# JuanLuisGonzalez/FAL_net

Measured on AMD Instinct MI355X. Metric: stereo-pairs/sec Stage-1 step @256x512 N=49, higher is better.
Workload: dtype bf16; 1 GPU; Stage-1 training step (BASELINE configs[1]), batch 8/GPU, 256x512, N=49, seeded weights, seeded VGG19; global_batch=8, parallelism=dp1, launch=eager launches, recorded sequences issued by falnet_replay (C)

## Files before the change

### fal_net_amd/_build.py

```python
import os
import subprocess
import sys
from concurrent.futures import ThreadPoolExecutor

HERE = os.path.dirname(os.path.abspath(__file__))
CSRC = os.path.join(HERE, "csrc")
OBJ = os.path.join(HERE, "csrc", "_obj")
LIB = os.path.join(HERE, "libfalnet_hip.so")
SOURCES = ["api.cpp", "replay.cpp", "med_head.hip", "med_head2.hip", "med_sweep.hip", "med_stats.hip", "compact.hip", "losses.hip", "elementwise.hip", "data.hip", "augment_batch.hip", "dump.hip", "metrics.hip", "velo.hip", "lidar.hip", "sort.hip", "sparsify.hip", "wgrad_rows.hip", "wgrad_wave.hip", "wgrad.hip", "pack.hip", "conv_wave.hip", "conv_dma.hip", "conv.hip"]
HIPCC = os.environ.get("HIPCC", "/opt/rocm/bin/hipcc")
FLAGS = ["--offload-arch=gfx950", "-O3", "-fPIC", "-std=c++17", "-Wall", "-Wno-unused-function"]
FILE_FLAGS = {"med_head.hip": ["-fno-slp-vectorize"], "med_head2.hip": ["-fno-slp-vectorize"], "med_sweep.hip": ["-fno-slp-vectorize"],
              "med_stats.hip": ["-fno-slp-vectorize"],
              "dump.hip": ["-ffp-contract=off"],
              "metrics.hip": ["-ffp-contract=off"], "augment_batch.hip": ["-ffp-contract=off"], "velo.hip": ["-ffp-contract=off"],
              "lidar.hip": ["-ffp-contract=off"], "sparsify.hip": ["-ffp-contract=off"]}


def _stale(out, deps):
    if not os.path.exists(out):
        return True
    t = os.path.getmtime(out)
    return any(os.path.getmtime(d) > t for d in deps)


def build_ab(tag="ab", defines=(), verbose=True, raw=()):
    obj_dir = os.path.join(CSRC, "_obj_" + tag)
    os.makedirs(obj_dir, exist_ok=True)
    flags = FLAGS + ["-DFALNET_AB"] + ["-D" + d for d in defines]
    lib = os.path.join(HERE, f"libfalnet_hip_{tag}.so")

    def run(src):
        cmd = [HIPCC] + flags + FILE_FLAGS.get(src, []) + list(raw) + (["-x", "hip"] if src.endswith(".hip") else []) + ["-c", os.path.join(CSRC, src), "-o", os.path.join(obj_dir, src + ".o")]
        if verbose:
            print(" ".join(cmd), flush=True)
        subprocess.run(cmd, check=True)
    with ThreadPoolExecutor(max_workers=4) as ex:
        list(ex.map(run, SOURCES))
    subprocess.run([HIPCC, "--offload-arch=gfx950", "-shared", "-fPIC", "-o", lib] + [os.path.join(obj_dir, s + ".o") for s in SOURCES], check=True)
    return lib


def build(force=False, verbose=True):
    os.makedirs(OBJ, exist_ok=True)
    headers = [os.path.join(CSRC, "common.h"), os.path.join(CSRC, "conv_epilogue.h"), os.path.join(HERE, "..", "include", "falnet_hip.h")]
    jobs = []
    for src in SOURCES:
        path = os.path.join(CSRC, src)
        obj = os.path.join(OBJ, src + ".o")
        if force or _stale(obj, [path] + headers):
            cmd = [HIPCC] + FLAGS + FILE_FLAGS.get(src, []) + (["-x", "hip"] if src.endswith(".hip") else []) + ["-c", path, "-o", obj]
            jobs.append(cmd)

    def run(cmd):
        if verbose:
            print(" ".join(cmd), flush=True)
        subprocess.run(cmd, check=True)

    with ThreadPoolExecutor(max_workers=4) as ex:
        list(ex.map(run, jobs))
    objs = [os.path.join(OBJ, s + ".o") for s in SOURCES]
    if force or jobs or _stale(LIB, objs):
        run([HIPCC, "--offload-arch=gfx950", "-shared", "-fPIC", "-o", LIB] + objs)
    return LIB


if __name__ == "__main__":
    if "--ab" in sys.argv:
        rest = [a for a in sys.argv[sys.argv.index("--ab") + 1:]]
        tag = next((a for a in rest if not a.startswith("-")), "ab")
        print(build_ab(tag, [a[2:] for a in rest if a.startswith("-D")], raw=[a for a in rest if a.startswith("-") and not a.startswith("-D")]))
    else:
        build(force="--force" in sys.argv)
        print(LIB)
```

### fal_net_amd/csrc/conv.hip

```cpp
#include <limits.h>
#include <stdlib.h>
#include <type_traits>
#include "common.h"
#include "conv_epilogue.h"

#define CONV_THREADS 256
#define CONV_BM 128
#define ROWB 64
#define ROWP 80

template <typename T> struct KC;
template <> struct KC<float> { static constexpr int value = 16; };
template <> struct KC<bf16_t> { static constexpr int value = 32; };
template <> struct KC<f16_t> { static constexpr int value = 32; };

template <typename T, int MT, int NT, typename RowOff, typename PoolOff = NoPool>
__device__ __forceinline__ void epilogue_nhwc(const falnet_conv_t& p, f32x16 (&acc)[MT][NT], float* stage, int nbase, int lane,
                                              RowOff rowoff, PoolOff pooloff = PoolOff()) {
    constexpr bool POOL = !std::is_same<PoolOff, NoPool>::value;
    constexpr int PITCHF = NT * 32 + 4;
    constexpr int CS = NT * 4;
    constexpr int RPP = 64 / CS;
    constexpr int PASSES = 32 / RPP;
    const int r = lane & 31, h = lane >> 5;
// ... 1382 lines not shown
    }
    C3_STAMP(5);
    asm volatile("s_waitcnt vmcnt(0)" ::: "memory");
    C3_STAMP(6);
}
#undef C3_STAMP

template <typename T, bool SWAP>
static void launch_conv(const falnet_conv_t& p, int bn, dim3 grid, hipStream_t st) {
    if (bn == 128)
        hipLaunchKernelGGL(HIP_KERNEL_NAME(conv_igemm_kernel<T, 128, SWAP>), grid, dim3(CONV_THREADS), 0, st, p);
    else if (bn == 64)
        hipLaunchKernelGGL(HIP_KERNEL_NAME(conv_igemm_kernel<T, 64, SWAP>), grid, dim3(CONV_THREADS), 0, st, p);
    else
        hipLaunchKernelGGL(HIP_KERNEL_NAME(conv_igemm_kernel<T, 32, SWAP>), grid, dim3(CONV_THREADS), 0, st, p);
}

static bool falnet_mfma16_enabled() {
    static const bool on = [] { const char* e = falnet_ab_env("FALNET_MFMA16"); return !(e && e[0] == '0'); }();
    return on;
}

enum class ConvFamily {
    Gather,
    Patch,
    WeightStationary,
    Dma,
    S2fDma,
    Up2Dma,
    Deep,
    Dma2,
    Dma16,
    Up2d,
    Wave32,
    Wave64p,
};
struct ConvChoice {
    ConvFamily family;
    int bn, kcb, tps, adb, th, nwaves, flip, swap;
};

static bool g_disable_patch = [] { const char* e = falnet_ab_env("FALNET_DISABLE_PATCH"); return e && e[0] == '1'; }();
static int g_patch_kcb = [] { const char* e = falnet_ab_env("FALNET_PATCH_KCB"); return e ? atoi(e) : 128; }();


bool falnet_conv_dma_applicable(const falnet_conv_t& p, int min_oh);
int falnet_conv_dma_launch(const falnet_conv_t& p, int flip, hipStream_t st, int th);
bool falnet_conv_dma2_applicable(const falnet_conv_t& p, int th);
int falnet_conv_dma2_launch(const falnet_conv_t& p, int flip, hipStream_t st, int th);
int falnet_conv_dma16_launch(const falnet_conv_t& p, int flip, hipStream_t st, int th);
bool falnet_conv_up2_dma_applicable(const falnet_conv_t& p);
int falnet_conv_up2_dma_launch(const falnet_conv_t& p, hipStream_t st);
bool falnet_conv_wave32_applicable(const falnet_conv_t& p);
int falnet_conv_wave32_launch(const falnet_conv_t& p, int flip, hipStream_t st);
bool falnet_conv_wave64p_applicable(const falnet_conv_t& p);
int falnet_conv_wave64p_launch(const falnet_conv_t& p, int flip, hipStream_t st);
bool falnet_conv_up2d_applicable(const falnet_conv_t& p);
int falnet_conv_up2d_launch(const falnet_conv_t& p, hipStream_t st);
bool falnet_conv_deep_applicable(const falnet_conv_t& p);
int falnet_conv_deep_launch(const falnet_conv_t& p, hipStream_t st);
int falnet_conv_deep_mtiles(const falnet_conv_t& p);
bool falnet_conv_s2d_dma_applicable(const falnet_conv_t* d, int n);
int falnet_conv_s2d_dma_launch(const falnet_conv_t* d, hipStream_t st);
bool falnet_conv_s2f_dma_applicable(const falnet_conv_t& p);
int falnet_conv_s2f_dma_launch(const falnet_conv_t& p, hipStream_t st);

static int choose_conv_kernel(const falnet_conv_t& p, ConvChoice& c) {
    const bool planar = p.out_layout == FALNET_OUT_PLANAR_F32;
    int ctot = 0;
    for (int s = 0; s < p.nsrc; ++s) ctot += p.src[s].C;
    bool dense3x3 = p.ntaps == 9 && p.isy == 1 && p.isx == 1 && p.osy == 1 && p.osx == 1 && p.ooy == 0 && p.oox == 0 &&
                    p.TH == p.OH && p.TW == p.OW && p.TH == p.IH && p.TW == p.IW && p.TW >= 16;
    int flip = -1;
    if (dense3x3 && p.w_taps == 9) {
        bool fwd = true, bwd = true;
        for (int t = 0; t < 9; ++t) {
            const int sp = (p.tap_dy[t] + 1) * 3 + (p.tap_dx[t] + 1);
            if (p.tap_dy[t] < -1 || p.tap_dy[t] > 1 || p.tap_dx[t] < -1 || p.tap_dx[t] > 1) fwd = bwd = false;
            fwd = fwd && p.tap_w[t] == sp;
            bwd = bwd && p.tap_w[t] == 8 - sp;
        }
        flip = fwd ? 0 : (bwd ? 1 : -1);
    }
    dense3x3 = dense3x3 && flip >= 0;
    const int esz = p.dtype == FALNET_F32 ? 4 : 2;
    bool c128 = true;
    for (int s = 0; s < p.nsrc; ++s) c128 = c128 && (p.src[s].C % (128 / esz) == 0);
    int variant = p.variant;
    int forced_bn = 0;
    if (variant == 11 || variant == 12) {
        forced_bn = variant == 11 ? 32 : 64;
        if (p.w_rows % forced_bn != 0 || p.pool_out) {
            falnet_set_error("conv2d: variant %d (gather, %d channels per workgroup) not applicable to this launch", variant, forced_bn);
            return -2;
        }
        variant = 1;
    }
    if (p.pool_code && !(variant == 23 && p.dtype != FALNET_F32 && p.pool_out && p.pool_mode == 0 && !planar && p.OH % 2 == 0 && p.OW % 2 == 0 &&
                         p.Cout % 32 == 0 && p.out_cstride % 32 == 0)) {
        falnet_set_error("conv2d: pool_code (argmax codes of the fused max pool) needs variant 23, a 16-bit type, pool_out with pool_mode 0, an NHWC "
                         "launch with even OH / OW and whole 32-channel groups (variant %d, dtype %d, pool_mode %d)", p.variant, p.dtype, p.pool_mode);
        return -2;
    }
    if (g_disable_patch) variant = 1;
    switch (variant) {
        case 0: case 1: case 2: case 3: case 4: case 5: case 6: case 7: case 8: case 9: case 10:
        case 13: case 15: case 16: case 17: case 18: case 19: case 20: case 21: case 22: case 23: case 24: case 25: case 26: case 27: case 29:
            break;
        default:
            falnet_set_error("conv2d: unknown variant %d", variant);
            return -1;
    }
    if (variant == 19) {
        if (!falnet_conv_deep_applicable(p)) {
            falnet_set_error("conv2d: variant 19 needs a 16-bit nine-tap stride-1/2 launch on maps of at most 128 positions (128 %% (TH TW) == 0), dense NHWC output, "
                             "w_rows %% 64 == 0, ksplit = cin_total / 32 or / 64 (a multiple of 4), scratch for the partial tiles and the split-K workspace");
            return -2;
        }
        c.flip = 0;
        c.swap = 0;
        c.family = ConvFamily::Deep;
        c.bn = 64; c.kcb = p.ksplit * 32 == p.cin_total ? 1 : 2; c.tps = 9; c.adb = 1; c.th = 0; c.nwaves = falnet_conv_deep_mtiles(p);
        return 0;
    }
    if (variant == 15) {
        if (!falnet_conv_s2f_dma_applicable(p)) {
            falnet_set_error("conv2d: variant 15 needs a canonical 16-bit 3x3 stride-2 pad-1 NHWC launch (>= 8 x 32 outputs) with sources at the input size");
            return -2;
        }
        c.flip = 0;
        c.swap = 0;
        c.family = ConvFamily::S2fDma;
        c.bn = 64; c.kcb = 32; c.tps = 9; c.adb = 1; c.th = 8; c.nwaves = 8;
        return 0;
    }
    if (variant == 29) {
        if (!(dense3x3 && falnet_conv_wave64p_applicable(p))) {
            falnet_set_error("conv2d: variant 29 needs a 16-bit dense 3x3 stride-1 launch over ONE 64-channel source at the launch size, planar f32 output of <= 4 channels, no addend / activation-gradient operand / pool / split-K");
            return -2;
        }
        c.flip = flip;
        c.swap = 0;
        c.family = ConvFamily::Wave64p;
        c.bn = 16; c.kcb = 32; c.tps = 9; c.adb = 1; c.th = 1; c.nwaves = 8;
        return 0;
    }
    if (variant == 27) {
        if (!(dense3x3 && falnet_conv_wave32_applicable(p))) {
            falnet_set_error("conv2d: variant 27 needs a 16-bit dense 3x3 stride-1 NHWC launch over ONE 32-channel source at the launch size with a 32-row packed weight, no pool / split-K");
            return -2;
        }
        c.flip = flip;
        c.swap = 0;
        c.family = ConvFamily::Wave32;
        c.bn = 32; c.kcb = 32; c.tps = 9; c.adb = 1; c.th = 1; c.nwaves = 8;
        return 0;
    }
    if (variant == 26) {
        if (!(falnet_conv_up2d_applicable(p) && p.ntaps == 4 && p.isy == 1 && p.isx == 1 && p.osy == 1 && p.osx == 1 && p.ooy == 0 && p.oox == 0 && p.TH == p.OH && p.TW == p.OW)) {
            falnet_set_error("conv2d: variant 26 needs a 16-bit NHWC launch over ONE source at exactly twice the output map (>= 16 x 32), w_taps = ntaps = 4, cin_total = 4 C, no pool / split-K");
            return -2;
        }
        c.flip = 0;
        c.swap = 0;
        c.family = ConvFamily::Up2d;
        c.bn = 64; c.kcb = 32; c.tps = 4; c.adb = 1; c.th = 16; c.nwaves = 8;
// ... 188 lines not shown
#undef LAUNCH_WS1
#undef LAUNCH_WS2
    return 0;
}

static int ws_symbol(char* buf, int len, const char* t, const falnet_conv_t& p, const ConvChoice& c) {
    const int m16 = (int)(falnet_mfma16_enabled() && p.dtype != FALNET_F32);
    if (c.adb) return snprintf(buf, len, "_Z18conv3x3_ws2_kernelI%sLi%dELi%dELb%dELb%dEEv13falnet_conv_tiii", t, c.bn, c.kcb, m16, (int)(c.kcb == 2 && ws2_whole_lines(p)));
    return snprintf(buf, len, "_Z17conv3x3_ws_kernelI%sLi%dELi%dELb%dEEv13falnet_conv_tiii", t, c.bn, c.kcb, m16);
}

struct ConvFamilyRow {
    ConvFamily family;
    int (*symbol)(char* buf, int len, const char* t, const falnet_conv_t& p, const ConvChoice& c);
    int (*launch)(const falnet_conv_t& p, const ConvChoice& c, hipStream_t st);
};
#define SYMBOL(...) [](char* buf, int len, const char* t, const falnet_conv_t& p, const ConvChoice& c) { return snprintf(buf, len, __VA_ARGS__); }
#define LAUNCH(...) [](const falnet_conv_t& p, const ConvChoice& c, hipStream_t st) { return __VA_ARGS__; }
static const ConvFamilyRow conv_families[] = {
    {ConvFamily::Gather, SYMBOL("_Z17conv_igemm_kernelI%sLi%dELb%dEEv13falnet_conv_t", t, c.bn, c.swap), launch_gather},
    {ConvFamily::Patch, SYMBOL("_Z20conv3x3_patch_kernelI%sLi%dELi%dELi%dELb%dELi%dELi%dEEv13falnet_conv_tiii", t, c.bn, c.kcb, c.tps, c.adb, c.th, c.nwaves), launch_patch},
    {ConvFamily::WeightStationary, ws_symbol, launch_ws},
    {ConvFamily::Dma, SYMBOL("_Z18conv3x3_dma_kernelI%sLi%dELi%dEEv13falnet_conv_tiiii", t, c.th, c.nwaves), LAUNCH(falnet_conv_dma_launch(p, c.flip, st, c.th))},
    {ConvFamily::S2fDma, SYMBOL("_Z22conv3x3_s2f_dma_kernelI%sLi%dEEv13falnet_conv_tiii", t, c.bn), LAUNCH(falnet_conv_s2f_dma_launch(p, st))},
    {ConvFamily::Up2Dma, SYMBOL("_Z22conv3x3_up2_dma_kernelI%sEv13falnet_conv_tiiiii", t), LAUNCH(falnet_conv_up2_dma_launch(p, st))},
    {ConvFamily::Deep, SYMBOL("_Z19conv3x3_deep_kernelI%sLi%dELi%dEEv13falnet_conv_t18falnet_deep_geom_t", t, c.kcb, c.nwaves), LAUNCH(falnet_conv_deep_launch(p, st))},
    {ConvFamily::Dma2, SYMBOL("_Z19conv3x3_dma2_kernelI%sLb%dELi%dEEv13falnet_conv_tiiiii", t, p.pool_out ? 1 : 0, c.nwaves), LAUNCH(falnet_conv_dma2_launch(p, c.flip, st, c.th))},
    {ConvFamily::Dma16, [](char* buf, int len, const char* t, const falnet_conv_t& p, const ConvChoice& c) {
         if (p.pool_out && p.pool_code) return snprintf(buf, len, "_Z20conv3x3_dma16_kernelI9PoolCodesI%sELb1ELi16ELi8ELb0EEv13falnet_conv_tiiii", t);
         return snprintf(buf, len, "_Z20conv3x3_dma16_kernelI%sLb%dELi%dELi%dELb%dEEv13falnet_conv_tiiii", t, p.pool_out ? 1 : 0, c.th, c.nwaves, p.out_layout == FALNET_OUT_PLANAR_F32 ? 1 : 0);
     },
     LAUNCH(falnet_conv_dma16_launch(p, c.flip, st, c.th))},
    {ConvFamily::Up2d, SYMBOL("_Z25conv2x2_up2d_dma16_kernelI%sEv13falnet_conv_tiii", t), LAUNCH(falnet_conv_up2d_launch(p, st))},
    {ConvFamily::Wave32, SYMBOL("_Z21conv3x3_wave32_kernelI%sEv13falnet_conv_tiiii", t), LAUNCH(falnet_conv_wave32_launch(p, c.flip, st))},
    {ConvFamily::Wave64p, SYMBOL("_Z22conv3x3_wave64p_kernelI%sEv13falnet_conv_tiiii", t), LAUNCH(falnet_conv_wave64p_launch(p, c.flip, st))},
};
#undef SYMBOL
#undef LAUNCH

static const ConvFamilyRow* conv_family_row(ConvFamily f) {
    for (const ConvFamilyRow& r : conv_families)
        if (r.family == f) return &r;
    falnet_set_error("conv2d: kernel family %d has no table row", (int)f);
    return nullptr;
}

extern "C" int falnet_conv2d_kernel_name(const falnet_conv_t* pp, char* buf, int len) {
    FALNET_CHECK_ARG(pp && buf && len > 0, "conv2d_kernel_name: bad argument");
    ConvChoice c;
    if (int r = choose_conv_kernel(*pp, c)) return r;
    const ConvFamilyRow* row = conv_family_row(c.family);
    if (!row) return -1;
    row->symbol(buf, len, pp->dtype == FALNET_BF16 ? "DF16b" : pp->dtype == FALNET_F16 ? "DF16_" : "f", *pp, c);
    return 0;
}

extern "C" int falnet_conv2d(const falnet_conv_t* pp, void* stream) {
    FALNET_ENTER(stream);
    FALNET_CHECK_ARG(pp, "conv2d: null descriptor");
    const falnet_conv_t& p = *pp;
    FALNET_CHECK_ARG(p.dtype == FALNET_F32 || p.dtype == FALNET_BF16 || p.dtype == FALNET_F16, "conv2d: bad dtype %d", p.dtype);
    const int kc = p.dtype == FALNET_F32 ? 16 : 32;
    FALNET_CHECK_ARG(p.nsrc == 1 || p.nsrc == 2, "conv2d: nsrc=%d", p.nsrc);
    int ctot = 0;
    for (int s = 0; s < p.nsrc; ++s) {
        if (int r = check_src(p.src[s], kc, "conv2d")) return r;
// ... 117 lines not shown
```

### fal_net_amd/csrc/conv_dma.hip

```cpp
#include <stdlib.h>
#include "conv_epilogue.h"

#ifndef FALNET_DMA_ROW_REUSE
#define FALNET_DMA_ROW_REUSE 1
#endif
#ifndef FALNET_DMA_EPI_AHEAD
#define FALNET_DMA_EPI_AHEAD -1
#endif
#ifndef FALNET_DMA16_EPI_AHEAD
#define FALNET_DMA16_EPI_AHEAD 0
#endif

#define CD_ZERO_BYTES 32768
__device__ uint4 g_cd_zero[CD_ZERO_BYTES / 16] = {};

typedef __attribute__((address_space(3))) void* cd_lptr_t;

__device__ __forceinline__ void cd_glds16(const void* gsrc, unsigned lds_dst) {
    unsigned keep;
    asm volatile("s_mov_b32 %0, m0\n\ts_mov_b32 m0, %2\n\ts_nop 0\n\tglobal_load_lds_dwordx4 %1, off\n\ts_mov_b32 m0, %0"
                 : "=&s"(keep)
                 : "v"(gsrc), "s"(lds_dst)
                 : "memory");
}

#define CD_PW 34

template <typename T, int TH, int NWAVES>
__global__ __launch_bounds__(NWAVES * 64) void conv3x3_dma_kernel(const falnet_conv_t p, int tiles_x, int tiles_y, int flip, int ntiles) {
    constexpr int BN = 64, MT = TH / NWAVES, NT = BN / 32;
    static_assert((MT == 1 || MT == 2) && sizeof(T) == 2, "one or two 32-position rows per wave, 16-bit operands");
    constexpr int KCV = 32;
    constexpr int NPIX = (TH + 2) * CD_PW;
    constexpr int A_PIECES = (NPIX + 15) / 16, B_PIECES = 9 * BN / 16, NPIECES = A_PIECES + B_PIECES;
// ... 2011 lines not shown
bool falnet_conv_s2f_dma_applicable(const falnet_conv_t& p) {
    if (p.dtype != FALNET_BF16 && p.dtype != FALNET_F16) return false;
    if (p.ntaps != 9 || p.w_taps != 9 || p.isy != 2 || p.isx != 2 || p.osy != 1 || p.osx != 1 || p.ooy || p.oox) return false;
    if (p.out_layout != FALNET_OUT_NHWC || p.pool_out || p.ksplit > 1 || p.nsrc < 1 || p.nsrc > 2) return false;
    for (int t = 0; t < 9; ++t)
        if (p.tap_dy[t] != t / 3 - 1 || p.tap_dx[t] != t % 3 - 1 || p.tap_w[t] != t) return false;
    if (p.TH != p.OH || p.TW != p.OW || p.OH != (p.IH + 1) / 2 || p.OW != (p.IW + 1) / 2 || p.OH < 8 || p.OW < 32) return false;
    for (int s = 0; s < p.nsrc; ++s) {
        const falnet_src_t& S = p.src[s];
        if (S.C % 16 || S.C <= 0 || S.H != p.IH || S.W != p.IW) return false;
        if ((int64_t)S.H * S.sy >= (1ll << 31)) return false;
    }
    if ((int64_t)p.w_rows * 9 * p.cin_total >= (1ll << 31) || (p.cin_total + 64) * 2 > CD_ZERO_BYTES) return false;
    return true;
}

int falnet_conv_s2f_dma_launch(const falnet_conv_t& p, hipStream_t st) {
    const int tiles_x = (p.OW + 31) / 32, tiles_y = (p.OH + 7) / 8;
    const int ntiles = p.B * tiles_x * tiles_y;
    static const bool allow128 = [] { const char* e = falnet_ab_env("FALNET_S2F_BN128"); return e && e[0] == '1'; }();
    const bool wide = allow128 && p.w_rows % 128 == 0 && p.Cout > 64;
    const int bn = wide ? 128 : 64;
    const int ny = (p.Cout + bn - 1) / bn;
    int gx = 256 / ny;
    if (gx < 1) gx = 1;
    if (gx > ntiles) gx = ntiles;
    const dim3 grid((unsigned)gx, (unsigned)ny);
#define SF_L(T) do { if (wide) hipLaunchKernelGGL(HIP_KERNEL_NAME(conv3x3_s2f_dma_kernel<T, 128>), grid, dim3(512), 0, st, p, tiles_x, tiles_y, ntiles); \
                     else hipLaunchKernelGGL(HIP_KERNEL_NAME(conv3x3_s2f_dma_kernel<T, 64>), grid, dim3(512), 0, st, p, tiles_x, tiles_y, ntiles); } while (0)
    FALNET_DISPATCH_16(p.dtype, SF_L);
#undef SF_L
    FALNET_RETURN_LAUNCH();
}
```

### fal_net_amd/ops.py

```python
import ctypes as C
import os
import sys

import torch

from . import _lib as L

CPAD = L.CPAD
H16 = (torch.bfloat16, torch.float16)
TYPE_SYM = {torch.bfloat16: "DF16b", torch.float16: "DF16_", torch.float32: "f"}

TIMER = None
AUTOTUNE = os.environ.get("FALNET_AUTOTUNE", "1") != "0"
DETERMINISTIC = L.DETERMINISTIC
UP2W = L.ab("FALNET_UP2W", "0") == "1"
UP2D = L.ab("FALNET_UP2D", "1") == "1"


_PKG_CACHE = os.path.join(os.path.dirname(os.path.abspath(__file__)), "autotune_cache.json")
_CACHE_PATH = os.environ.get("FALNET_AUTOTUNE_CACHE", _PKG_CACHE)
_CACHE_WRITABLE = ("FALNET_AUTOTUNE_CACHE" in os.environ and _CACHE_PATH != "0") or os.environ.get("FALNET_AUTOTUNE_CACHE_WRITE") == "1"
_GATES = {"FALNET_NO_DMA": "0", "FALNET_WS2": "1", "FALNET_S2F_DMA": "1", "FALNET_S2D_DMA": "1", "FALNET_S2_SPLITK": "1",
          "FALNET_GATHER_NARROW": "0", "FALNET_S2_MULTI": None, "FALNET_SMALL_TILE_DMA": "1", "FALNET_UP2": "1", "FALNET_DEEP": "1", "FALNET_TILE8": "1"}
if os.environ.get("FALNET_AB") == "1" and any(os.environ.get(k, v) != v for k, v in _GATES.items()):
    _CACHE_PATH = "0"
_CACHE = None
_CACHE_DIRTY = False
_TUNE_SOURCES = ("conv.hip", "conv_dma.hip", "conv_wave.hip", "conv_epilogue.h", "common.h")


def cache_meta():
    import hashlib
    h = hashlib.sha256()
    csrc = os.path.join(os.path.dirname(os.path.abspath(__file__)), "csrc")
    for name in _TUNE_SOURCES:
        path = os.path.join(csrc, name)
        if os.path.isfile(path):
            with open(path, "rb") as f:
                h.update(name.encode() + b"\0" + f.read())
    return {"src_hash": h.hexdigest()[:16], "version": int(L.lib().falnet_version()), "arch": "gfx950"}


def _cache():
    global _CACHE
    if _CACHE is None:
        _CACHE = {}
        if _CACHE_PATH != "0" and os.path.isfile(_CACHE_PATH):
            try:
                import json
                with open(_CACHE_PATH) as f:
                    data = json.load(f)
                if data.pop("_meta", None) == cache_meta():
                    _CACHE = data
                elif os.environ.get("FALNET_AUTOTUNE_LOG") == "1":
                    print(f"[autotune] {_CACHE_PATH}: tuned with another build of the kernels -- ignored", file=sys.stderr)
# ... 438 lines not shown
    wgs = ((M + 127) // 128) * ((Cout + bn - 1) // bn)
    if wgs < 256 and M * w_rows * 4 <= d.splitk_ws_bytes and Cout % 8 == 0:
        cands += [(1, k) for k in (2, 4, 8, 16) if wgs * k <= 2048]
    if wgs < 256 and GATHER_NARROW:
        for v, nb in ((12, 64), (11, 32)):
            if nb < bn and w_rows % nb == 0:
                w2 = ((M + 127) // 128) * ((Cout + nb - 1) // nb)
                cands += [(v, 1)]
                if M * w_rows * 4 <= d.splitk_ws_bytes and Cout % 8 == 0:
                    cands += [(v, k) for k in (2, 4) if w2 * k <= 2048]
    cands += [(2, 1), (3, 1), (4, 1), (6, 1), (7, 1), (10, 1)]
    if L.ab("FALNET_WS2", "1") == "1":
        cands += [(16, 1)]
    if L.ab("FALNET_NO_DMA", "0") != "1":
        cands += [(13, 1)]
        if L.ab("FALNET_DMA2", "0") == "1":
            cands += [(21, 1), (22, 1)]
        if L.ab("FALNET_DMA16", "1") == "1":
            cands += [(23, 1)]
            if wgs < int(L.ab("FALNET_SMALL_TILE_MAXWGS", "1024")):
                cands += [(24, 1), (25, 1)]
        if d.cin_total == 32 and w_rows == 32 and L.ab("FALNET_CONV_WAVE", "1") == "1":
            cands += [(27, 1)]
        if d.cin_total == 64 and d.out_layout == L.OUT_PLANAR_F32 and Cout <= 4 and L.ab("FALNET_CONV_WAVE", "1") == "1":
            cands += [(29, 1)]
        if d.weight_up2:
            cands += [(18, 1)]
        if wgs < int(L.ab("FALNET_SMALL_TILE_MAXWGS", "1024")) and L.ab("FALNET_SMALL_TILE_DMA", "1") == "1":
            cands += [(17, 1)]
            if L.ab("FALNET_TILE8", "1") == "1":
                cands += [(20, 1)]
        if d.isy == 2 and L.ab("FALNET_S2F_DMA", "1") == "1":
            cands += [(15, 1)]
    if wgs < 512:
        cands += [(8, 1), (9, 1)]
    if d.TH * d.TW <= 128 and d.ntaps == 9 and L.ab("FALNET_DEEP", "1") == "1":
        cands += [(19, d.cin_total // kc) for kc in (32, 64) if d.cin_total % (4 * kc) == 0]
    best, best_t = (1, 1), None
    for v, k in cands:
        d.variant, d.ksplit = v, k
        if lib.falnet_conv2d(ref, st) != 0:
            if _AUTOTUNE_LOG:
                print(f"[autotune] M={M} w_rows={w_rows} Cout={Cout} v{v} k{k}: n/a ({lib.falnet_last_error().decode()}) "
                      f"src={[(d.src[i].C, d.src[i].H, d.src[i].W) for i in range(d.nsrc)]} cin_total={d.cin_total}", file=sys.stderr)
            continue
        lib.falnet_conv2d(ref, st)
        t = None
        for _ in range(3):
            e0, e1 = torch.cuda.Event(enable_timing=True), torch.cuda.Event(enable_timing=True)
            e0.record()
            for _ in range(reps):
                lib.falnet_conv2d(ref, st)
            e1.record()
            e1.synchronize()
            tt = e0.elapsed_time(e1)
            t = tt if t is None else min(t, tt)
        if _AUTOTUNE_LOG:
            print(f"[autotune] M={M} w_rows={w_rows} Cout={Cout} ntaps={d.ntaps} nsrc={d.nsrc} v{v} k{k}: {t / reps * 1e3:.1f} us", file=sys.stderr)
        if best_t is None or t < best_t:
            best, best_t = (v, k), t
    return best


def _wgrad_plan(dtype, srcs, taps, stride_in, B, TH, TW, IH, IW, cin_pad, cout_pad, max_slabs, target_wgs=1536, up2=False):
    M = B * TH * TW
    h16 = dtype in (torch.bfloat16, torch.float16)
# ... 334 lines not shown
```

Measured before the change: 1643 stereo-pairs/s.

## Add parity-plane stride-2 3x3 conv kernel as autotune candidate

Adds a new forward 3x3 stride-2 convolution kernel that splits the input into four parity planes (even/odd rows and columns), so each chunk stages a dense tile via DMA-to-LDS and runs only the taps that apply to that plane with 16x16 MFMA. It also folds per-sample constant sources (spatially broadcast channels) into a precomputed border-aware bias instead of staging them. The kernel is registered as variants 30/31 (tile heights 16 and 8) and added to the autotuner's candidate list for stride-2 layers. The autotuner keeps it only if it times faster, at the cost of more code and compile time.

```diff
diff --git a/fal_net_amd/_build.py b/fal_net_amd/_build.py
--- a/fal_net_amd/_build.py
+++ b/fal_net_amd/_build.py
@@ -43,7 +43,7 @@
 
 def build(force=False, verbose=True):
     os.makedirs(OBJ, exist_ok=True)
-    headers = [os.path.join(CSRC, "common.h"), os.path.join(CSRC, "conv_epilogue.h"), os.path.join(HERE, "..", "include", "falnet_hip.h")]
+    headers = [os.path.join(CSRC, "common.h"), os.path.join(CSRC, "conv_epilogue.h"), os.path.join(CSRC, "conv_s2p_host.h"), os.path.join(HERE, "..", "include", "falnet_hip.h")]
     jobs = []
     for src in SOURCES:
         path = os.path.join(CSRC, src)
diff --git a/fal_net_amd/csrc/conv.hip b/fal_net_amd/csrc/conv.hip
--- a/fal_net_amd/csrc/conv.hip
+++ b/fal_net_amd/csrc/conv.hip
@@ -1438,6 +1438,7 @@
     Dma2,
     Dma16,
     Up2d,
+    S2Planes,
     Wave32,
     Wave64p,
 };
@@ -1470,6 +1471,9 @@
 int falnet_conv_s2d_dma_launch(const falnet_conv_t* d, hipStream_t st);
 bool falnet_conv_s2f_dma_applicable(const falnet_conv_t& p);
 int falnet_conv_s2f_dma_launch(const falnet_conv_t& p, hipStream_t st);
+const char* falnet_conv_s2p_why_not(const falnet_conv_t& p, int th);
+bool falnet_conv_s2p_const_plane(const falnet_conv_t& p);
+int falnet_conv_s2p_launch(const falnet_conv_t& p, hipStream_t st, int th);
 
 static int choose_conv_kernel(const falnet_conv_t& p, ConvChoice& c) {
     const bool planar = p.out_layout == FALNET_OUT_PLANAR_F32;
@@ -1511,7 +1515,7 @@
     if (g_disable_patch) variant = 1;
     switch (variant) {
         case 0: case 1: case 2: case 3: case 4: case 5: case 6: case 7: case 8: case 9: case 10:
-        case 13: case 15: case 16: case 17: case 18: case 19: case 20: case 21: case 22: case 23: case 24: case 25: case 26: case 27: case 29:
+        case 13: case 15: case 16: case 17: case 18: case 19: case 20: case 21: case 22: case 23: case 24: case 25: case 26: case 27: case 29: case 30: case 31:
             break;
         default:
             falnet_set_error("conv2d: unknown variant %d", variant);
@@ -1538,6 +1542,18 @@
         c.swap = 0;
         c.family = ConvFamily::S2fDma;
         c.bn = 64; c.kcb = 32; c.tps = 9; c.adb = 1; c.th = 8; c.nwaves = 8;
+        return 0;
+    }
+    if (variant == 30 || variant == 31) {
+        const int th = variant == 30 ? 16 : 8;
+        if (const char* why = falnet_conv_s2p_why_not(p, th)) {
+            falnet_set_error("conv2d: variant %d (3x3 stride-2 forward by parity plane, %d x 32 tiles) needs %s", variant, th, why);
+            return -2;
+        }
+        c.flip = 0;
+        c.swap = 0;
+        c.family = ConvFamily::S2Planes;
+        c.bn = 64; c.kcb = 32; c.tps = 4; c.adb = 1; c.th = th; c.nwaves = 8;
         return 0;
     }
     if (variant == 29) {
@@ -1792,6 +1808,7 @@
      },
      LAUNCH(falnet_conv_dma16_launch(p, c.flip, st, c.th))},
     {ConvFamily::Up2d, SYMBOL("_Z25conv2x2_up2d_dma16_kernelI%sEv13falnet_conv_tiii", t), LAUNCH(falnet_conv_up2d_launch(p, st))},
+    {ConvFamily::S2Planes, SYMBOL("_Z24conv3x3_s2p_dma16_kernelI%sLi%dELb%dEEv13falnet_conv_tiiiiii", t, c.th / 8, (int)falnet_conv_s2p_const_plane(p)), LAUNCH(falnet_conv_s2p_launch(p, st, c.th))},
     {ConvFamily::Wave32, SYMBOL("_Z21conv3x3_wave32_kernelI%sEv13falnet_conv_tiiii", t), LAUNCH(falnet_conv_wave32_launch(p, c.flip, st))},
     {ConvFamily::Wave64p, SYMBOL("_Z22conv3x3_wave64p_kernelI%sEv13falnet_conv_tiiii", t), LAUNCH(falnet_conv_wave64p_launch(p, c.flip, st))},
 };
diff --git a/fal_net_amd/csrc/conv_dma.hip b/fal_net_amd/csrc/conv_dma.hip
--- a/fal_net_amd/csrc/conv_dma.hip
+++ b/fal_net_amd/csrc/conv_dma.hip
@@ -1,5 +1,6 @@
 #include <stdlib.h>
 #include "conv_epilogue.h"
+#include "conv_s2p_host.h"
 
 #ifndef FALNET_DMA_ROW_REUSE
 #define FALNET_DMA_ROW_REUSE 1
@@ -2077,3 +2078,355 @@
 #undef SF_L
     FALNET_RETURN_LAUNCH();
 }
+
+template <typename T, int MT, bool CP>
+__global__ __launch_bounds__(512) void conv3x3_s2p_dma16_kernel(const falnet_conv_t p, int tiles_x, int tiles_y, int ntiles, int s0, int s1, int cs) {
+    constexpr int TH = 8 * MT, NWAVES = 8, BN = 64, NT = 2, KCV = 32;
+    constexpr int NPIX = (TH + 1) * CD_PW;
+    constexpr int A_PIECES = (NPIX + 15) / 16, B_PIECES = 4 * BN / 16, NPIECES = A_PIECES + B_PIECES;
+    constexpr int A_BYTES = A_PIECES * 1024, BUF = NPIECES * 1024;
+    constexpr int ROWB = CD_PW * 64;
+    __shared__ __attribute__((aligned(1024))) char lds[2 * BUF];
+    __shared__ __attribute__((aligned(16))) float lds_bias[BN];
+    __shared__ __attribute__((aligned(16))) float lds_ts[CP ? 9 * BN : 4], lds_cv[CP ? 9 * BN : 4];
+    const int tid = threadIdx.x, lane = tid & 63;
+    const int wave = __builtin_amdgcn_readfirstlane(tid >> 6);
+    const unsigned lds_base = (unsigned)(unsigned long)(cd_lptr_t)lds;
+    const int r = lane & 31;
+    const int lp = lane & 15, lg = lane >> 4;
+    const int n0 = blockIdx.y * BN;
+    const char* const zero_page = reinterpret_cast<const char*>(g_cd_zero);
+    stage_bias_lds(p, n0, BN, lds_bias);
+
+    const int IH = p.IH, IW = p.IW;
+    const falnet_src_t& S0 = s0 == 0 ? p.src[0] : p.src[1];
+    const falnet_src_t& S1 = s1 < 0 ? S0 : (s1 == 0 ? p.src[0] : p.src[1]);
+    const T* const sp0 = reinterpret_cast<const T*>(S0.ptr);
+    const T* const sp1 = reinterpret_cast<const T*>(S1.ptr);
+    const int k0 = s0 == 0 ? 0 : p.src[0].C, k1 = s1 <= 0 ? 0 : p.src[0].C;
+    const int nc0 = S0.C / KCV;
+    const int cpc = nc0 + (s1 < 0 ? 0 : S1.C / KCV);
+    const int nchunks = 4 * cpc;
+    int my_tiles = 0;
+    for (int t = blockIdx.x; t < ntiles; t += gridDim.x) ++my_tiles;
+    const int total = my_tiles * nchunks;
+
+    constexpr int KP = (A_PIECES + NWAVES - 1) / NWAVES, KW = B_PIECES / NWAVES, NP = KP + KW;
+    static_assert(B_PIECES == KW * NWAVES, "every wave issues KW weight pieces");
+    const int l4 = lane >> 2, segpos = lane & 3;
+    const T* const wptr = reinterpret_cast<const T*>(p.weight);
+    const T* const zero_t = reinterpret_cast<const T*>(zero_page);
+    int w_base[KW];
+#pragma unroll
+    for (int k = 0; k < KW; ++k) {
+        const int wid = wave + NWAVES * k;
+        const int co = n0 + ((wid & 3) << 4) + l4;
+        const int gseg = segpos ^ (((l4 >> 2) & 1) << 1);
+        w_base[k] = co < p.w_rows ? co * 9 * p.cin_total + gseg * 8 : -1;
+    }
+    struct TPos { int b, ty, tx; };
+    TPos step_;
+    {
+        const int g = (int)gridDim.x;
+        step_.tx = g % tiles_x;
+        const int q = g / tiles_x;
+        step_.ty = q % tiles_y;
+        step_.b = q / tiles_y;
+    }
+    auto pos_of = [&](int tile) {
+        TPos t;
+        t.tx = tile % tiles_x;
+        const int q = tile / tiles_x;
+        t.ty = q % tiles_y;
+        t.b = q / tiles_y;
+        return t;
+    };
+    auto pos_next = [&](TPos& t) {
+        t.tx += step_.tx;
+        if (t.tx >= tiles_x) { t.tx -= tiles_x; ++t.ty; }
+        t.ty += step_.ty;
+        if (t.ty >= tiles_y) { t.ty -= tiles_y; ++t.b; }
+        t.b += step_.b;
+    };
+    int prc_[KP], a_off[KP];
+#pragma unroll
+    for (int k = 0; k < KP; ++k) {
+        const int pix = 16 * (wave + NWAVES * k) + l4;
+        const int pr = pix / CD_PW, pc = pix - pr * CD_PW;
+        prc_[k] = ((pix < NPIX && pc <= 32) ? pr : (1 << 20)) << 8 | pc;
+        a_off[k] = 2 * pr * (int)S0.sy + 2 * pc * (int)S0.sx + (segpos ^ (((pc >> 2) & 1) << 1)) * 8;
+    }
+    unsigned a_ok = 0, t_ok = 0;
+    const T* a_base = sp0;
+    int f_e = 0, f_f = 0, f_kofs = 0;
+    struct Cur { int tile, cin, ord; TPos t; };
+    auto chunk_setup = [&](const Cur& q) {
+        const int ef = (0x2103 >> (4 * q.ord)) & 3;
+        const int e = ef >> 1, f = ef & 1;
+        const int second = q.cin >= nc0 ? 1 : 0;
+        const int c0 = (second ? q.cin - nc0 : q.cin) * KCV;
+        const int y0 = 2 * (q.t.ty * TH - 1) + e, x0 = 2 * (q.t.tx * 32 - 1) + f;
+        a_base = second ? sp1 + ((int64_t)q.t.b * S1.sb + (int64_t)y0 * (int)S1.sy + (int64_t)x0 * (int)S1.sx + c0)
+                        : sp0 + ((int64_t)q.t.b * S0.sb + (int64_t)y0 * (int)S0.sy + (int64_t)x0 * (int)S0.sx + c0);
+        f_e = e; f_f = f;
+        f_kofs = (second ? k1 : k0) + c0;
+        a_ok = t_ok >> (8 * ef);
+    };
+    static_assert(KP <= 8, "one byte of in-map bits per plane");
+    auto tile_setup = [&](const Cur& q) {
+        t_ok = 0;
+#pragma unroll
+        for (int ef = 0; ef < 4; ++ef) {
+            const int e = ef >> 1, f = ef & 1;
+            const int y0 = 2 * (q.t.ty * TH - 1) + e, x0 = 2 * (q.t.tx * 32 - 1) + f;
+#pragma unroll
+            for (int k = 0; k < KP; ++k) {
+                const int pr = prc_[k] >> 8, pc = prc_[k] & 255;
+                const int vy = y0 + 2 * pr, vx = x0 + 2 * pc;
+                const bool used = (e || pr > 0) && (f || pc > 0);
+                t_ok |= (used && vy >= 0 && vy < IH && vx >= 0 && vx < IW) ? 1u << (8 * ef + k) : 0u;
+            }
+        }
+    };
+    auto advance = [&](Cur& q) {
+        if (++q.ord == 4) {
+            q.ord = 0;
+            if (++q.cin == cpc) {
+                q.cin = 0;
+                q.tile += gridDim.x;
+                pos_next(q.t);
+                if (q.tile >= ntiles) return;
+                tile_setup(q);
+            }
+        }
+        chunk_setup(q);
+    };
+    auto issue_piece = [&](int buf, int i) {
+        const unsigned dst0 = lds_base + buf * BUF;
+        if (i < KP) {
+            const int id = wave + NWAVES * i;
+            const T* src = ((a_ok >> i) & 1) ? a_base + a_off[i] : zero_t;
+            if (id < A_PIECES) cd_glds16(src, dst0 + id * 1024);
+        } else {
+            const int k = i - KP;
+            const int wid = wave + NWAVES * k;
+            const int t = wid >> 2, du = t >> 1, dv = t & 1;
+            if ((f_e || du) && (f_f || dv)) {
+                const int tap = (f_e ? 2 * du : 1) * 3 + (f_f ? 2 * dv : 1);
+                const T* src = w_base[k] >= 0 ? wptr + (w_base[k] + tap * p.cin_total + f_kofs) : zero_t;
+                cd_glds16(src, dst0 + A_BYTES + wid * 1024);
+            }
+        }
+    };
+
+    int a_lane[2][2];
+#pragma unroll
+    for (int dv = 0; dv < 2; ++dv)
+#pragma unroll
+        for (int pt = 0; pt < 2; ++pt) {
+            const int col = dv + 16 * pt + lp;
+            a_lane[dv][pt] = ((wave * MT) * CD_PW + col) * 64 + ((lg ^ (((col >> 2) & 1) << 1)) << 4);
+        }
+    const int wrow = m16_row_channel(lp);
+    const int b_lane = A_BYTES + wrow * 64 + ((lg ^ (((wrow >> 2) & 1) << 1)) << 4);
+
+    Acc16 acc[MT][NT];
+#pragma unroll
+    for (int mt = 0; mt < MT; ++mt)
+#pragma unroll
+        for (int nt = 0; nt < NT; ++nt) acc[mt][nt].zero();
+    Cur qi = {(int)blockIdx.x, 0, 0, pos_of((int)blockIdx.x)};
+    TPos ct = qi.t;
+    if (total > 0) {
+        tile_setup(qi);
+        chunk_setup(qi);
+#pragma unroll
+        for (int i = 0; i < NP; ++i) issue_piece(0, i);
+        advance(qi);
+    }
+    const falnet_src_t& SC = cs == 1 ? p.src[1] : p.src[0];
+    const int kc = cs == 1 ? p.src[0].C : 0;
+    [[maybe_unused]] float cp_sa = 0.f, cp_sb = 0.f;
+    [[maybe_unused]] uint4 cw[2][2] = {}, cv4[2] = {};
+    [[maybe_unused]] auto cp_fetch = [&](int half) {
+        const int co = n0 + lane;
+        const T* wa = co < p.w_rows ? wptr + ((co * 9 + wave) * p.cin_total + kc + 16 * half) : zero_t;
+        const T* wb = co < p.w_rows ? wptr + ((co * 9 + 8) * p.cin_total + kc + 16 * half) : zero_t;
+        const T* vp = reinterpret_cast<const T*>(SC.ptr) + ((int64_t)ct.b * SC.sb + 16 * half);
+#pragma unroll
+        for (int j = 0; j < 2; ++j) {
+            cw[0][j] = reinterpret_cast<const uint4*>(wa)[j];
+            cw[1][j] = reinterpret_cast<const uint4*>(wb)[j];
+            cv4[j] = reinterpret_cast<const uint4*>(vp)[j];
+        }
+    };
+    if constexpr (CP) {
+        if (total > 0) cp_fetch(0);
+    }
+    int cc = 0;
+    for (int it = 0; it < total; ++it) {
+        asm volatile("s_waitcnt vmcnt(0) lgkmcnt(0)" ::: "memory");
+        __builtin_amdgcn_s_barrier();
+        const bool more = it + 1 < total;
+        const int nb = (it + 1) & 1;
+        int bo = (it & 1) * BUF;
+        asm volatile("" : "+s"(bo));
+        const char* const Bf = lds;
+        if constexpr (CP) {
+            if (cc < 2) {
+                float sa = cc ? cp_sa : 0.f, sb = cc ? cp_sb : 0.f;
+#pragma unroll
+                for (int j = 0; j < 2; ++j) {
+                    const unsigned wa[4] = {cw[0][j].x, cw[0][j].y, cw[0][j].z, cw[0][j].w}, wb[4] = {cw[1][j].x, cw[1][j].y, cw[1][j].z, cw[1][j].w};
+                    const unsigned vv[4] = {cv4[j].x, cv4[j].y, cv4[j].z, cv4[j].w};
+#pragma unroll
+                    for (int d = 0; d < 4; ++d) {
+                        sa = fmaf(H16<T>::lo(wa[d]), H16<T>::lo(vv[d]), sa);
+                        sa = fmaf(H16<T>::hi(wa[d]), H16<T>::hi(vv[d]), sa);
+                        sb = fmaf(H16<T>::lo(wb[d]), H16<T>::lo(vv[d]), sb);
+                        sb = fmaf(H16<T>::hi(wb[d]), H16<T>::hi(vv[d]), sb);
+                    }
+                }
+                cp_sa = sa;
+                cp_sb = sb;
+                if (cc == 1) {
+                    lds_ts[wave * BN + lane] = sa;
+                    if (wave == 0) lds_ts[8 * BN + lane] = sb;
+                }
+            } else if (cc == 2) {
+                for (int idx = tid; idx < 9 * BN; idx += NWAVES * 64) {
+                    const int cls = idx / BN, co = idx - cls * BN;
+                    const int rc = cls / 3, cl = cls - rc * 3;
+                    float s = 0.f;
+#pragma unroll
+                    for (int ky = 0; ky < 3; ++ky)
+#pragma unroll
+                        for (int kx = 0; kx < 3; ++kx) {
+                            const bool in = !(rc == 0 && ky == 0) && !(rc == 2 && ky == 2) && !(cl == 0 && kx == 0) && !(cl == 2 && kx == 2);
+                            s += in ? lds_ts[(ky * 3 + kx) * BN + co] : 0.f;
+                        }
+                    lds_cv[idx] = s;
+                }
+            }
+            __builtin_amdgcn_sched_barrier(0);
+        }
+        int aa[2][2];
+#pragma unroll
+        for (int dv = 0; dv < 2; ++dv)
+#pragma unroll
+            for (int pt = 0; pt < 2; ++pt) aa[dv][pt] = a_lane[dv][pt] + bo;
+        const int bb = b_lane + bo;
+        auto a_read = [&](int dv, int rs, int pt) { return *reinterpret_cast<const s16x8_t*>(Bf + aa[dv][pt] + rs * ROWB); };
+        auto mma_phase = [&](auto Ec, auto Fc) {
+            constexpr int E = decltype(Ec)::value, F = decltype(Fc)::value;
+            constexpr int NE = 1 + E, NS = NE * (1 + F), NSLOT = NS * MT, PER = (NP + NSLOT - 1) / NSLOT;
+            int slot = 0;
+#pragma unroll
+            for (int dv = 1 - F; dv < 2; ++dv) {
+                s16x8_t fa[MT + 1][2];
+#pragma unroll
+                for (int rs = 1 - E; rs <= MT; ++rs)
+#pragma unroll
+                    for (int pt = 0; pt < 2; ++pt) fa[rs][pt] = a_read(dv, rs, pt);
+#pragma unroll
+                for (int du = 1 - E; du < 2; ++du) {
+                    s16x8_t fb[NT][2];
+#pragma unroll
+                    for (int nt = 0; nt < NT; ++nt)
+#pragma unroll
+                        for (int ct2 = 0; ct2 < 2; ++ct2) fb[nt][ct2] = *reinterpret_cast<const s16x8_t*>(Bf + bb + ((2 * du + dv) * BN + nt * 32 + ct2 * 16) * 64);
+#pragma unroll
+                    for (int half = 0; half < MT; ++half) {
+                        if (more) {
+#pragma unroll
+                            for (int i = slot * PER; i < (slot + 1) * PER && i < NP; ++i) issue_piece(nb, i);
+                        }
+                        ++slot;
+#pragma unroll
+                        for (int nt = 0; nt < NT; ++nt)
+#pragma unroll
+                            for (int ct2 = 0; ct2 < 2; ++ct2)
+#pragma unroll
+                                for (int pt = 0; pt < 2; ++pt)
+                                    acc[half][nt].t[ct2][pt] = H16<T>::mma16(fb[nt][ct2], fa[half + du][pt], acc[half][nt].t[ct2][pt]);
+                    }
+                }
+            }
+        };
+        const int ord = it & 3;
+        if (ord == 0) mma_phase(std::integral_constant<int, 1>(), std::integral_constant<int, 1>());
+        else if (ord == 1) mma_phase(std::integral_constant<int, 0>(), std::integral_constant<int, 0>());
+        else if (ord == 2) mma_phase(std::integral_constant<int, 0>(), std::integral_constant<int, 1>());
+        else mma_phase(std::integral_constant<int, 1>(), std::integral_constant<int, 0>());
+        if (more) advance(qi);
+        if (++cc == nchunks) {
+            cc = 0;
+            const int b = ct.b, ty0 = ct.ty * TH, tx0 = ct.tx * 32;
+            pos_next(ct);
+            const int cstride = p.out_cstride;
+            const int x = tx0 + r;
+            const int64_t obase = (((int64_t)b * p.OH + ty0) * p.OW + tx0) * cstride;
+            auto pixoff = [&](int mt) -> int64_t {
+                const int y = ty0 + wave * MT + mt;
+                if (!(y < p.OH && x < p.OW)) return (int64_t)-1;
+                return obase + ((wave * MT + mt) * p.OW + r) * cstride;
+            };
+            const int h = lane >> 5;
+#pragma unroll
+            for (int nt = 0; nt < NT; ++nt) {
+                float bias[1][16];
+                load_bias16_lds(lds_bias, 32 * nt, h, bias);
+#pragma unroll
+                for (int mt = 0; mt < MT; ++mt) {
+                    f32x16 v[1][1];
+                    acc[mt][nt].to32(v[0][0]);
+                    acc[mt][nt].zero();
+                    if constexpr (CP) {
+                        const int y = ty0 + wave * MT + mt;
+                        const int rc = y == 0 ? 0 : (2 * y + 1 >= IH ? 2 : 1), cl = x == 0 ? 0 : (2 * x + 1 >= IW ? 2 : 1);
+                        const float* cvp = lds_cv + (rc * 3 + cl) * BN + 32 * nt + 4 * h;
+#pragma unroll
+                        for (int m = 0; m < 4; ++m) {
+                            const float4 c4 = *reinterpret_cast<const float4*>(cvp + 8 * m);
+                            v[0][0][4 * m + 0] += c4.x;
+                            v[0][0][4 * m + 1] += c4.y;
+                            v[0][0][4 * m + 2] += c4.z;
+                            v[0][0][4 * m + 3] += c4.w;
+                        }
+                    }
+                    auto pixoff1 = [&](int) -> int64_t { return pixoff(mt); };
+                    epilogue_direct<T, 1, 1, decltype(pixoff1), NoPool, -1, false, true>(p, v, bias, n0 + 32 * nt, lane, pixoff1);
+                }
+            }
+        }
+        if constexpr (CP) {
+            if (more && cc < 2) cp_fetch(cc);
+        }
+    }
+}
+
+bool falnet_conv_s2p_applicable(const falnet_conv_t& p, int th) { return falnet_s2p_why_not(p, th) == nullptr; }
+const char* falnet_conv_s2p_why_not(const falnet_conv_t& p, int th) { return falnet_s2p_why_not(p, th); }
+bool falnet_conv_s2p_const_plane(const falnet_conv_t& p) {
+    for (int s = 0; s < p.nsrc; ++s)
+        if (falnet_s2p_const_src(p.src[s])) return true;
+    return false;
+}
+
+int falnet_conv_s2p_launch(const falnet_conv_t& p, hipStream_t st, int th) {
+    const falnet_s2p_grid_t g = falnet_s2p_grid(p, th);
+    int s0 = -1, s1 = -1, cs = -1;
+    for (int s = 0; s < p.nsrc; ++s) {
+        if (cs < 0 && falnet_s2p_const_src(p.src[s])) cs = s;
+        else if (s0 < 0) s0 = s;
+        else s1 = s;
+    }
+    const dim3 grid((unsigned)g.gx, (unsigned)g.gy);
+#define S2P_K(T, MT_, CP_) hipLaunchKernelGGL(HIP_KERNEL_NAME(conv3x3_s2p_dma16_kernel<T, MT_, CP_>), grid, dim3(512), 0, st, p, g.tiles_x, g.tiles_y, g.ntiles, s0, s1, cs)
+#define S2P_L(T) do { if (th == 16) { if (cs >= 0) S2P_K(T, 2, true); else S2P_K(T, 2, false); } \
+                      else { if (cs >= 0) S2P_K(T, 1, true); else S2P_K(T, 1, false); } } while (0)
+    FALNET_DISPATCH_16(p.dtype, S2P_L);
+#undef S2P_L
+#undef S2P_K
+    FALNET_RETURN_LAUNCH();
+}
diff --git a/fal_net_amd/csrc/conv_s2p_host.h b/fal_net_amd/csrc/conv_s2p_host.h
--- /dev/null
+++ b/fal_net_amd/csrc/conv_s2p_host.h
@@ -0,0 +1,51 @@
+#pragma once
+#include <stdint.h>
+#include "../../include/falnet_hip.h"
+
+#define S2P_ZERO_BYTES 32768
+
+static inline bool falnet_s2p_const_src(const falnet_src_t& S) { return S.sy == 0 && S.sx == 0 && S.C == 32; }
+
+static inline const char* falnet_s2p_why_not(const falnet_conv_t& p, int th) {
+    if (th != 16 && th != 8) return "tile height must be 16 or 8";
+    if (p.dtype != FALNET_BF16 && p.dtype != FALNET_F16) return "a 16-bit type";
+    if (p.ntaps != 9 || p.w_taps != 9) return "nine taps";
+    if (p.isy != 2 || p.isx != 2 || p.osy != 1 || p.osx != 1 || p.ooy || p.oox) return "input stride 2, dense output";
+    for (int t = 0; t < 9; ++t)
+        if (p.tap_dy[t] != t / 3 - 1 || p.tap_dx[t] != t % 3 - 1 || p.tap_w[t] != t) return "the canonical 3x3 pad-1 tap table";
+    if (p.out_layout != FALNET_OUT_NHWC || p.pool_out || p.ksplit > 1 || !p.out) return "a plain NHWC output (no pool, no split-K)";
+    if (p.nsrc < 1 || p.nsrc > 2) return "one or two sources";
+    if (p.TH != p.OH || p.TW != p.OW || p.OH != (p.IH + 1) / 2 || p.OW != (p.IW + 1) / 2) return "OH x OW = ceil(IH / 2) x ceil(IW / 2) tile space";
+    if (p.OW < 32) return "OW >= 32";
+    if (p.OH < th) return th == 16 ? "OH >= 16 (variant 30)" : "OH >= 8 (variant 31)";
+    int ctot = 0, nreal = 0;
+    for (int s = 0; s < p.nsrc; ++s) {
+        const falnet_src_t& S = p.src[s];
+        if (S.C <= 0 || S.C % 32) return "every source a multiple of 32 channels";
+        if (S.H != p.IH || S.W != p.IW) return "sources at the input size";
+        if ((int64_t)S.H * S.sy + (int64_t)S.W * S.sx >= (1ll << 31)) return "a sample below 2^31 elements";
+        ctot += S.C;
+        nreal += falnet_s2p_const_src(S) ? 0 : 1;
+    }
+    if (nreal < 1) return "at least one source that is not constant per sample";
+    if (nreal == 2 && (p.src[0].sy != p.src[1].sy || p.src[0].sx != p.src[1].sx)) return "two staged sources with the same row and pixel strides";
+    if (ctot > p.cin_total) return "sources within the packed weight row";
+    if ((int64_t)p.w_rows * 9 * p.cin_total >= (1ll << 31)) return "a packed weight below 2^31 elements";
+    if ((p.cin_total + 64) * 2 > S2P_ZERO_BYTES) return "a weight row within the zero page";
+    return nullptr;
+}
+
+struct falnet_s2p_grid_t {
+    int tiles_x, tiles_y, ntiles, gx, gy;
+};
+static inline falnet_s2p_grid_t falnet_s2p_grid(const falnet_conv_t& p, int th) {
+    falnet_s2p_grid_t g;
+    g.tiles_x = (p.OW + 31) / 32;
+    g.tiles_y = (p.OH + th - 1) / th;
+    g.ntiles = p.B * g.tiles_x * g.tiles_y;
+    g.gy = (p.Cout + 63) / 64;
+    g.gx = 256 / g.gy;
+    if (g.gx < 1) g.gx = 1;
+    if (g.gx > g.ntiles) g.gx = g.ntiles;
+    return g;
+}
diff --git a/fal_net_amd/ops.py b/fal_net_amd/ops.py
--- a/fal_net_amd/ops.py
+++ b/fal_net_amd/ops.py
@@ -20,7 +20,7 @@
 _PKG_CACHE = os.path.join(os.path.dirname(os.path.abspath(__file__)), "autotune_cache.json")
 _CACHE_PATH = os.environ.get("FALNET_AUTOTUNE_CACHE", _PKG_CACHE)
 _CACHE_WRITABLE = ("FALNET_AUTOTUNE_CACHE" in os.environ and _CACHE_PATH != "0") or os.environ.get("FALNET_AUTOTUNE_CACHE_WRITE") == "1"
-_GATES = {"FALNET_NO_DMA": "0", "FALNET_WS2": "1", "FALNET_S2F_DMA": "1", "FALNET_S2D_DMA": "1", "FALNET_S2_SPLITK": "1",
+_GATES = {"FALNET_NO_DMA": "0", "FALNET_WS2": "1", "FALNET_S2F_DMA": "1", "FALNET_S2_PLANES": "1", "FALNET_S2D_DMA": "1", "FALNET_S2_SPLITK": "1",
           "FALNET_GATHER_NARROW": "0", "FALNET_S2_MULTI": None, "FALNET_SMALL_TILE_DMA": "1", "FALNET_UP2": "1", "FALNET_DEEP": "1", "FALNET_TILE8": "1"}
 if os.environ.get("FALNET_AB") == "1" and any(os.environ.get(k, v) != v for k, v in _GATES.items()):
     _CACHE_PATH = "0"
@@ -525,6 +525,8 @@
                 cands += [(20, 1)]
         if d.isy == 2 and L.ab("FALNET_S2F_DMA", "1") == "1":
             cands += [(15, 1)]
+        if d.isy == 2 and L.ab("FALNET_S2_PLANES", "1") == "1":
+            cands += [(30, 1), (31, 1)]
     if wgs < 512:
         cands += [(8, 1), (9, 1)]
     if d.TH * d.TW <= 128 and d.ntaps == 9 and L.ab("FALNET_DEEP", "1") == "1":
```

Result: no change. 1639 stereo-pairs/s (-0.2%).
